# idra-lab/safe-mpc

Hardware: AMD Instinct MI355X
Metric: RTI-MPC instance-steps/s (batch=4096 per GPU, Z1 N=30) (higher is better)
Workload: dtype f64; 1 GPU; C1: Z1-class 6-DoF, N=30, 4096 instances/GPU, controller st (soft terminal NN row, MLP 12-256-256-256-1 fp32), EXT cost exact Hessian, 6 capsule pairs, Halton x0; batch_per_gpu=4096, batch_total=4096, horizon=30, controller=st, streams_per_gpu=3, qp_form=throughput, hip_graphs=False

## Files before the change

include/smpc.h:

```cpp
#ifndef SMPC_H_
#define SMPC_H_

#include <stddef.h>
#include <stdint.h>

#ifdef __cplusplus
extern "C" {
#endif

#define SMPC_ABI_VERSION 5

#define SMPC_MAX_NQ 7
#define SMPC_MAX_NX 14
#define SMPC_MAX_POINTS 12
#define SMPC_MAX_ROWS 12
#define SMPC_MAX_LAYERS 6
#define SMPC_MAX_N 63
#define SMPC_NP 5

#define SMPC_INF 1.0e5

#define SMPC_OK 0
#define SMPC_EINVAL (-1)
#define SMPC_ENOMEM (-2)
// ... 90 lines not shown
} smpc_problem_desc;

typedef struct {
    double tau[SMPC_MAX_NQ];
    double M[SMPC_MAX_NQ * SMPC_MAX_NQ];
    double dtau_dq[SMPC_MAX_NQ * SMPC_MAX_NQ];
    double dtau_dv[SMPC_MAX_NQ * SMPC_MAX_NQ];
    double ee[3];
    double cost_grad_q[SMPC_MAX_NQ];
    double cost_hess_qq[SMPC_MAX_NQ * SMPC_MAX_NQ];
    double row_val[SMPC_MAX_ROWS];
    double row_grad[SMPC_MAX_ROWS * SMPC_MAX_NQ];
    double nn_val;
    double nn_grad[SMPC_MAX_NX];
} smpc_node_eval;

typedef struct smpc_handle smpc_handle;

int smpc_create(const smpc_problem_desc* desc, int device, smpc_handle** out);
void smpc_destroy(smpc_handle* h);
int smpc_abi_version(void);
const char* smpc_last_error(const smpc_handle* h);

int smpc_set_mlp(smpc_handle* h, int nlayers, const int32_t* dims, const float* const* W, const float* const* b,
                 int on_device);
enum { SMPC_ACT_GELU_TANH = 0, SMPC_ACT_RELU = 1, SMPC_ACT_ELU = 2, SMPC_ACT_TANH = 3, SMPC_ACT_SILU = 4 };
int smpc_set_mlp_activation(smpc_handle* h, int act);

int smpc_set_horizon(smpc_handle* h, int N);

enum { SMPC_QP_AUTO = -1, SMPC_QP_THROUGHPUT = 0, SMPC_QP_LATENCY = 1 };
int smpc_set_qp_mode(smpc_handle* h, int mode);

int smpc_set_stage_bounds(smpc_handle* h, const double* lo, const double* hi);

int smpc_set_instance_bounds(smpc_handle* h, int B, const double* lo, const double* hi, int on_device);

#define SMPC_SCENE_ROW 8
int smpc_set_instance_scene(smpc_handle* h, int B, const double* geom, int on_device);

int smpc_set_instance_scene_track(smpc_handle* h, int B, int64_t T, const double* geom, int on_device);

int smpc_set_scene_clock(smpc_handle* h, const int64_t* d_clock);

int smpc_set_instance_world_track(smpc_handle* h, int B, int64_t T, const double* geom, int on_device);

enum { SMPC_FORECAST_HOLD = 0, SMPC_FORECAST_CV = 1, SMPC_FORECAST_TRUE = 2 };
int smpc_forecast_scene(smpc_handle* h, int B, int mode, int n_sel, const int32_t* select);

int smpc_set_instance_observed_track(smpc_handle* h, int B, int64_t T, const double* geom, int on_device);

#define SMPC_FIT_MAX 32
int smpc_forecast_scene_fit(smpc_handle* h, int B, int window, int n_sel, const int32_t* select);

int smpc_set_instance_curves(smpc_handle* h, int B, int64_t L, const double* curves, int on_device);

int smpc_set_instance_models(smpc_handle* h, int B, const smpc_joint* joints, int on_device);

int smpc_set_mlp_context(smpc_handle* h, int n_ctx, const float* Wc, const double* ctx_mean, const double* ctx_std,
                         const double* ctx_default, int on_device);

int smpc_set_instance_context(smpc_handle* h, int B, const double* ctx, int on_device);

int smpc_set_instance_context_track(smpc_handle* h, int B, int64_t T, const double* ctx, int on_device);

int smpc_set_slack_weights(smpc_handle* h, const double* zl);
// ... 194 lines not shown
```

safe_mpc_amd/_lib.py:

```python
from __future__ import annotations

import ctypes as C
import os
import subprocess

from .problem import Joint, NodeEval, ProblemDesc

_CSRC = os.path.join(os.path.dirname(os.path.abspath(__file__)), 'csrc')
LIB_PATH = os.environ.get('SMPC_HIP_LIB') or os.path.join(_CSRC, 'libsmpc_hip.so')

SYMBOLS = ['smpc_create', 'smpc_destroy', 'smpc_abi_version', 'smpc_last_error', 'smpc_set_mlp', 'smpc_set_horizon',
           'smpc_set_stage_bounds', 'smpc_set_slack_weights', 'smpc_set_instance_bounds', 'smpc_solve_batch', 'smpc_eval_nodes', 'smpc_guess_correction',
           'smpc_provide_control', 'smpc_check_trajectory', 'smpc_plant_step', 'smpc_rollout_batch', 'smpc_sync', 'smpc_stream',
           'smpc_enable_timing', 'smpc_get_timing', 'smpc_get_qp_timing', 'smpc_get_qp_wave_stats', 'smpc_policy_step', 'smpc_loop_pre',
           'smpc_loop_post', 'smpc_loop_apply_backup', 'smpc_loop_classify_aborts', 'smpc_get_timing_history',
           'smpc_accumulate_stats', 'smpc_set_mlp_activation', 'smpc_set_qp_mode', 'smpc_merit_terms', 'smpc_sqp_batch', 'smpc_check_guess',
           'smpc_score_rollout', 'smpc_set_instance_scene', 'smpc_ik_batch', 'smpc_ray_update', 'smpc_set_instance_curves',
           'smpc_set_instance_scene_track', 'smpc_set_scene_clock', 'smpc_set_mlp_context', 'smpc_set_instance_context',
           'smpc_set_instance_models', 'smpc_set_instance_context_track', 'smpc_set_instance_world_track', 'smpc_forecast_scene',
           'smpc_set_instance_observed_track', 'smpc_forecast_scene_fit']


class EngineError(RuntimeError):
    pass


_vp = C.c_void_p


class PolicyParams(C.Structure):
    _fields_ = [('kind', C.c_int32), ('abort_flag', C.c_int32), ('collision_first_node', C.c_int32), ('reserved0', C.c_int32),
                ('tol_x', C.c_double), ('alpha', C.c_double), ('tol_safe', C.c_double), ('tube', C.c_double),
                ('x_min', _vp), ('x_max', _vp), ('row_lb_chk', _vp), ('row_ub_chk', _vp), ('stage_lo', _vp), ('stage_hi', _vp)]


class PolicyState(C.Structure):
    _fields_ = [(k, _vp) for k in ('x_guess', 'u_guess', 'x_temp', 'u_temp', 'p', 'x_viable', 'fails', 'current_step', 'r',
                                   'status', 'qp_iter', 'traj')] + [('traj_len', C.c_int64)]


class LoopState(C.Structure):
    _fields_ = [(k, _vp) for k in ('x_cur', 'alive', 'sa', 'collided', 'ja', 'last_x', 'last_u', 'x_abort', 'u_abort', 'step',
                                   'x_log', 'u_log', 'r_log', 'resumed')]


class SqpOpts(C.Structure):
    _fields_ = [('max_iter', C.c_int32), ('reserved0', C.c_int32), ('tol', C.c_double), ('armijo', C.c_double),
                ('alpha_reduction', C.c_double), ('alpha_min', C.c_double), ('mu0', C.c_double), ('mu_max', C.c_double)]

# ... 75 lines not shown
    L.smpc_set_instance_world_track.argtypes = [vp, C.c_int, C.c_int64, dp, C.c_int]
    L.smpc_forecast_scene.argtypes = [vp, C.c_int, C.c_int, C.c_int, dp]
    L.smpc_set_instance_observed_track.argtypes = [vp, C.c_int, C.c_int64, dp, C.c_int]
    L.smpc_forecast_scene_fit.argtypes = [vp, C.c_int, C.c_int, C.c_int, dp]
    L.smpc_set_instance_curves.argtypes = [vp, C.c_int, C.c_int64, dp, C.c_int]
    L.smpc_solve_batch.argtypes = [vp, C.c_int, dp, dp, dp, dp, dp, dp, dp, dp, C.c_int]
    L.smpc_eval_nodes.argtypes = [vp, C.c_int, dp, dp, dp, dp, C.c_int]
    L.smpc_guess_correction.argtypes = [vp, C.c_int, dp, dp, C.c_int]
    L.smpc_provide_control.argtypes = [vp, C.c_int, dp, dp, dp, dp, dp, dp, C.c_int]
    L.smpc_check_trajectory.argtypes = [vp, C.c_int, C.c_int, dp, dp, dp, C.c_double, dp, dp, C.c_double, C.c_double,
                                        dp, dp, C.c_int]
    L.smpc_plant_step.argtypes = [vp, C.c_int, dp, dp, dp, dp, dp, dp, C.c_int]
    L.smpc_rollout_batch.argtypes = [vp, C.c_int, C.c_int, dp, dp, dp, dp, dp, dp, dp, dp, dp, dp, C.c_int]
    L.smpc_sync.argtypes = [vp]
    L.smpc_stream.argtypes = [vp]
    L.smpc_stream.restype = C.c_void_p
    L.smpc_enable_timing.argtypes = [vp, C.c_int]
    L.smpc_get_timing.argtypes = [vp, C.POINTER(C.c_float)]
    L.smpc_get_qp_timing.argtypes = [vp, C.POINTER(C.c_float)]
    L.smpc_get_qp_wave_stats.argtypes = [vp, C.POINTER(C.c_double)]
    L.smpc_policy_step.argtypes = [vp, C.c_int, C.POINTER(PolicyParams), C.POINTER(PolicyState), dp, dp, dp, dp, dp, dp]
    L.smpc_loop_pre.argtypes = [vp, C.c_int, C.c_int, C.POINTER(LoopState), dp, dp, dp, dp]
    L.smpc_loop_apply_backup.argtypes = [vp, C.c_int, C.c_int, C.POINTER(LoopState), C.c_int, dp, dp, dp, dp, dp, dp, dp]
    L.smpc_loop_post.argtypes = [vp, C.c_int, C.POINTER(PolicyParams), C.POINTER(LoopState), dp, dp, dp]
    L.smpc_loop_classify_aborts.argtypes = [vp, C.c_int, C.POINTER(LoopState), C.c_int, dp, dp]
    L.smpc_get_timing_history.argtypes = [vp, C.c_int, C.POINTER(C.c_float)]
    L.smpc_accumulate_stats.argtypes = [vp, C.c_int, dp, dp, dp]
    L.smpc_set_mlp_activation.argtypes = [vp, C.c_int]
    L.smpc_set_mlp_context.argtypes = [vp, C.c_int, dp, dp, dp, dp, C.c_int]
    L.smpc_set_instance_context.argtypes = [vp, C.c_int, dp, C.c_int]
    L.smpc_set_instance_context_track.argtypes = [vp, C.c_int, C.c_int64, dp, C.c_int]
    L.smpc_set_instance_models.argtypes = [vp, C.c_int, dp, C.c_int]
    L.smpc_set_qp_mode.argtypes = [vp, C.c_int]
    L.smpc_merit_terms.argtypes = [vp, C.c_int, dp, dp, dp, dp, dp, dp, dp, dp, dp, C.c_int]
    L.smpc_sqp_batch.argtypes = [vp, C.c_int, C.POINTER(SqpOpts), dp, dp, dp, dp, C.POINTER(SqpState), C.c_int]
    L.smpc_check_guess.argtypes = [vp, C.c_int, dp, dp, C.POINTER(GuessCheck), dp, dp, dp, C.c_int]
    L.smpc_score_rollout.argtypes = [vp, C.c_int, C.c_int, dp, dp, dp, dp, C.POINTER(ScoreParams), dp, dp, dp, C.c_int]
    L.smpc_ik_batch.argtypes = [vp, C.c_int, C.c_int, dp, dp, C.POINTER(IkParams), dp, dp, dp, dp, C.c_int]
    L.smpc_ray_update.argtypes = [vp, C.c_int, C.POINTER(RayOpts), C.POINTER(RayState), C.POINTER(SqpState), dp, dp, dp, dp, dp, C.c_int]
    _lib = L
    return L
```

safe_mpc_amd/csrc/engine.hip:

```cpp
#include <hip/hip_runtime.h>

#include <cstdarg>
#include <cstdio>
#include <cstring>
#include <new>
#include <type_traits>
#include <vector>

#include "../../include/smpc.h"
#include "kernel_qp.hpp"
#include "kernel_qp_wg.hpp"
#include "kernel_build.hpp"
#include "kernels_callers.hpp"
#include "kernels_policy.hpp"
#include "kernels_mlp.hpp"
#include "kernels_nodes.hpp"
#include "kernels_sqp.hpp"
#include "kernels_guess.hpp"
#include "kernels_score.hpp"
#include "kernels_ik.hpp"
#include "kernels_rays.hpp"
#include "kernels_forecast.hpp"

using namespace smpc;
// ... 58 lines not shown
    smpc_problem_desc desc;
    int device = 0;
    int N = 0;
    hipStream_t stream = nullptr;
    smpc_problem_desc* d_desc = nullptr;
    DevBuf<double> d_lo, d_hi;
    DevBuf<double> d_zl;
    InstSlot<double> bounds{"per-instance bounds", "smpc_set_instance_bounds"};
    InstSlot<double> scene{"instance scene", "smpc_set_instance_scene"};
    int64_t scene_T = 1;
    const int64_t* scene_clock = nullptr;
    bool scene_fc = false;
    InstSlot<double> world{"instance world track", "smpc_set_instance_world_track"};
    int64_t world_T = 1;
    InstSlot<double> seen{"instance observed track", "smpc_set_instance_observed_track"};
    int64_t seen_T = 1;
    InstSlot<double> curves{"instance curve table", "smpc_set_instance_curves"};
    int64_t curves_L = 0;
    InstSlot<float> ctx{"instance context", "smpc_set_instance_context"};
    int64_t ctx_T = 1;
    bool ctx_fc = false;
    InstSlot<smpc_joint> models{"instance model table", "smpc_set_instance_models"};
    Net own_net;
    const Net* net = &own_net;
    DevBuf<double> d_ev;
    DevBuf<double> d_nn;
    DevBuf<double> d_ws;
    int qp_mode = -2;
    DevBuf<double> d_hrec;
    bool wg_lds_raised[2] = {false, false};
    DevBuf<int32_t> d_order, d_last_it;
    int order_B = 0;
    DevBuf<int32_t> d_ord_hist;
    DevBuf<float> d_S, d_y, d_GS, d_dA, d_dB;
    DevBuf<int32_t> d_nn_idx;
    int32_t* d_nn_cnt = nullptr;
    DevBuf<float> d_act[SMPC_MAX_LAYERS];
    DevBuf<float> d_dg[SMPC_MAX_LAYERS];
    DevBuf<char> d_stage;
    ParamBlock chk{"check bounds"};
    ParamBlock gchk{"guess check bounds"};
    ParamBlock schk{"score bounds"};
    ParamBlock ikb{"inverse kinematics bounds"};
    DevBuf<char> d_roll;
    int timing = 0;
    int timed = 0;
    static constexpr int EV_RING = 64;
    hipEvent_t ev_sets[EV_RING][5] = {};
    bool ev_complete[EV_RING] = {};
    hipEvent_t* ev_t = ev_sets[0];
    int ev_cur = 0;
    bool timing_now = false;
    long timed_count = 0;
    std::vector<smpc_handle*> kids;
    hipEvent_t ev_fork = nullptr, ev_join = nullptr;
    DevBuf<unsigned long long> d_wstat;
    const uint8_t* d_active = nullptr;
    DevBuf<char> d_polw;
    float last_ms[4] = {0, 0, 0, 0};
    long mlp_rows_whole = 0;
    long mlp_rows_hint = 0;
    DevBuf<char> d_par;
    DevBuf<char> d_sqp;
    DevBuf<int32_t> d_guess;
    DevBuf<char> d_score;
    char err[256] = "";
// ... 345 lines not shown
    }
    if (st->traj) {
        if (st->traj_len < 1) return fail(h, SMPC_EINVAL, "traj_len must be >= 1");
        *out = TrajSrc{st->traj, (long)st->traj_len, 0};
    }
    return SMPC_OK;
}

template <int NQ>
int launch_eval(smpc_handle* h, int B, const double* d_xg, const double* d_ug, const double* d_p, double* d_ev) {
    const int N = h->N;
    hipStream_t s = h->stream;
    const long n1 = (long)B * (N + 1);
    with_scene(h, B, [&](auto SCENE, auto sc) {
        return with_model(h, B, [&](auto MODEL, auto... md) {
            hipLaunchKernelGGL((k_node_linearise<NQ, SCENE, MODEL>), dim3((unsigned)((n1 + 63) / 64)), dim3(64), 0, s, h->d_desc, B, N, d_xg,
                               d_ug, d_p, d_ev, sc, md...);
            return SMPC_OK;
        });
    });
    HIPCHK(h, hipGetLastError());
    int rc;
    if ((rc = launch_nn<NQ>(h, B, d_xg, d_p, d_ev, 0))) return rc;
    if (h->desc.nn_mode == SMPC_NN_ALL && h->d_nn_cnt) HIPCHK(h, hipMemsetAsync(h->d_nn_cnt, 0, sizeof(int32_t), s));
    return SMPC_OK;
}

constexpr size_t qp_nt_threshold = (size_t)384 << 20;
static int qp_nt_mode() {
    static const int v = [] { const char* e = getenv("SMPC_QP_NT"); return e ? atoi(e) : -1; }();
    return v;
}

template <class F> int with_rows(const smpc_handle* h, F&& f) {
    switch (h->desc.n_rows) {
    case 6: return f(std::integral_constant<int, 6>{});
    case 4: return f(std::integral_constant<int, 4>{});
    default: return f(std::integral_constant<int, -1>{});
    }
}

int ensure_instance_bounds(smpc_handle* h, int B, bool zero) { return h->bounds.room(h, (size_t)2 * B * (h->N + 1) * 2 * h->desc.nq, zero); }
double* instance_hi(const smpc_handle* h) { return h->bounds.d.p ? h->bounds.d.p + h->bounds.d.cap / (2 * sizeof(double)) : nullptr; }

struct StageBounds {
    const double *lo, *hi;
    long stride;
};
StageBounds stage_bounds(const smpc_handle* h, int B) {
    if (const double* lo = h->bounds.for_batch(B)) return {lo, instance_hi(h), (long)(h->N + 1) * 2 * h->desc.nq};
    return {h->d_lo.p, h->d_hi.p, 0L};
}

template <int NQ>
int launch_stage_records(smpc_handle* h, int B, const double* x0, const double* xg, const double* ug, const double* p, bool timed) {
    int rc;
    if ((rc = launch_nn<NQ>(h, B, xg, p, h->d_nn.p, h->desc.nn_mode == SMPC_NN_TERMINAL ? 2 : 1))) return rc;
    if (timed) HIPCHK(h, hipEventRecord(h->ev_t[1], h->stream));
    const StageBounds bd = stage_bounds(h, B);
    const long nodes = (long)B * (h->N + 1);
    const dim3 grd((unsigned)((nodes + 64 / SB_G - 1) / (64 / SB_G))), blk(64);
    const double* nn = h->desc.nn_mode != SMPC_NN_NONE ? h->d_nn.p : nullptr;
    int32_t* const zero_cnt = h->desc.nn_mode == SMPC_NN_ALL ? h->d_nn_cnt : nullptr;
    with_rows(h, [&](auto MR) {
        return with_scene(h, B, [&](auto SCENE, auto sc) {
            return with_model(h, B, [&](auto MODEL, auto... md) {
// ... 93 lines not shown
        h->timing_now = !capturing(h);
    }
    const bool timed = h->timing_now;
    if (timed) {
        h->ev_cur = (h->ev_cur + 1) % smpc_handle::EV_RING;
        h->ev_t = h->ev_sets[h->ev_cur];
        h->ev_complete[h->ev_cur] = false;
        h->timed_count++;
        HIPCHK(h, hipEventRecord(h->ev_t[0], h->stream));
    }
    if ((rc = launch_stage_records<NQ>(h, B, x0, xg, ug, p, timed))) return rc;
    const int wg_nhw = qp_wg_choice<NQ>(h, B);
    const bool wg = wg_nhw > 0;
    const int32_t* order = nullptr;
    if (h->order_B == B && B > 1 && !wg) {
        hipLaunchKernelGGL(k_order_by_iters, dim3((B + ORD_PER_BLOCK - 1) / ORD_PER_BLOCK), dim3(64), 0, h->stream, B, h->d_last_it.p,
                           h->d_order.p, h->d_ord_hist.p, h->d_ord_hist.p + 256, h->d_ord_hist.p + 512);
        order = h->d_order.p;
    } else {
        HIPCHK(h, hipMemsetAsync(h->d_ord_hist.p, 0, 520 * sizeof(int32_t), h->stream));
    }
    unsigned long long* wstat = nullptr;
    if (timed && h->timing == 1) {
        const unsigned long long init[4] = {0ull, ~0ull, 0ull, 0ull};
        HIPCHK(h, hipMemcpyAsync(h->d_wstat.p, init, sizeof(init), hipMemcpyHostToDevice, h->stream));
        wstat = h->d_wstat.p;
    }
    if (wg) {
        if ((rc = wg_nhw == 8 ? launch_qp_wg<NQ, 8>(h, B, x0, xg, ug, xo, uo, st, it) : launch_qp_wg<NQ, 4>(h, B, x0, xg, ug, xo, uo, st, it))) return rc;
    } else {
        const bool nt = qp_nt_mode() < 0 ? ws_doubles_per_instance(h, h->N) * sizeof(double) * (size_t)B >= qp_nt_threshold : qp_nt_mode() > 0;
        with_rows(h, [&](auto MR) {
            const auto launch = [&](auto NT) {
                hipLaunchKernelGGL((k_qp_ipm<NQ, MR, NT>), dim3((B + 1) / 2), dim3(64), 0, h->stream, h->d_desc, B, h->N, x0, xg, ug, h->d_ws.p,
                                   xo, uo, st, it, order, h->d_last_it.p, wstat, h->d_active, h->d_ord_hist.p);
                return SMPC_OK;
            };
            if constexpr (MR < 0) return launch(std::false_type{});
            else return nt ? launch(std::true_type{}) : launch(std::false_type{});
        });
    }
    h->order_B = B;
    HIPCHK(h, hipGetLastError());
    if (timed) {
        HIPCHK(h, hipEventRecord(h->ev_t[3], h->stream));
        h->ev_complete[h->ev_cur] = true;
        h->timed = 1;
    }
    return SMPC_OK;
}

struct ChkBlock { double *x_min, *x_max, *row_lb, *row_ub; size_t doubles; };
ChkBlock chk_block(double* base, int nq) {
    Carve m = dense(base);
    ChkBlock b{};
    b.x_min = m.take<double>(2 * nq);
    b.x_max = m.take<double>(2 * nq);
    b.row_lb = m.take<double>(SMPC_MAX_ROWS);
    b.row_ub = m.take<double>(SMPC_MAX_ROWS);
    b.doubles = m.off / sizeof(double);
    return b;
}
int upload_check_bounds(smpc_handle* h, const double* x_min, const double* x_max, const double* row_lb_chk,
                        const double* row_ub_chk) {
    const int nq = h->desc.nq, nr = h->desc.n_rows;
    std::vector<double> img(chk_block(nullptr, nq).doubles, 0.0);
    const ChkBlock b = chk_block(img.data(), nq);
    put(b.x_min, x_min, 2 * nq);
// ... 65 lines not shown
    return SMPC_OK;
}

struct RollScratch {
    int32_t *fails, *accept, *it;
    double *xo, *uo;
    size_t bytes;
};
RollScratch roll_layout(char* base, int n, int N, int nq) {
    Carve m{base};
    RollScratch r{};
    r.fails = m.take<int32_t>(n);
    r.accept = m.take<int32_t>(n);
    r.xo = m.take<double>((size_t)n * (N + 1) * 2 * nq);
    r.uo = m.take<double>((size_t)n * N * nq);
    r.it = m.take<int32_t>(n);
    r.bytes = m.off;
    return r;
}

int rollout_workers(smpc_handle* h, int n) {
    while ((int)h->kids.size() < n) {
        smpc_handle* k = nullptr;
        int rc = smpc_create(&h->desc, h->device, &k);
        if (rc) return fail(h, rc, "rollout worker: %s", smpc_last_error(nullptr));
        h->kids.push_back(k);
    }
    for (int i = 0; i < n; i++) {
        smpc_handle* k = h->kids[i];
        int rc;
        if (k->N != h->N && (rc = smpc_set_horizon(k, h->N))) return fail(h, rc, "rollout worker: %s", k->err);
        k->net = h->net;
        k->qp_mode = h->qp_mode;
        const size_t nb = (size_t)(h->N + 1) * 2 * h->desc.nq;
        HIPCHK(h, hipMemcpyAsync(k->d_lo.p, h->d_lo.p, nb * sizeof(double), hipMemcpyDeviceToDevice, k->stream));
        HIPCHK(h, hipMemcpyAsync(k->d_hi.p, h->d_hi.p, nb * sizeof(double), hipMemcpyDeviceToDevice, k->stream));
        if (h->d_zl.p) {
            if ((rc = k->d_zl.reserve(k, "slack weights", sizeof(double) * (h->N + 1)))) return fail(h, rc, "rollout worker: %s", k->err);
            HIPCHK(h, hipMemcpyAsync(k->d_zl.p, h->d_zl.p, sizeof(double) * (h->N + 1), hipMemcpyDeviceToDevice, k->stream));
        } else if (k->d_zl.p) {
            HIPCHK(h, hipStreamSynchronize(k->stream));
            k->d_zl.release();
        }
    }
    return SMPC_OK;
}

struct ParScratch {
    double *p1, *x0, *xg, *ug, *p, *xo, *uo;
    int32_t *st, *it, *ok, *safe, *list, *pos, *n_open;
    uint8_t* active;
    size_t bytes;
};
ParScratch par_layout(char* base, int B, int N, int nq) {
    const size_t S = (size_t)B * (N - 1), nx = 2 * (size_t)nq;
    Carve m{base};
    ParScratch c{};
    c.p1 = m.take<double>((size_t)B * (N + 1) * SMPC_NP);
    c.x0 = m.take<double>(S * nx);
    c.xg = m.take<double>(S * (N + 1) * nx);
    c.ug = m.take<double>(S * N * nq);
    c.p = m.take<double>(S * (N + 1) * SMPC_NP);
    c.xo = m.take<double>(S * (N + 1) * nx);
    c.uo = m.take<double>(S * N * nq);
    c.st = m.take<int32_t>(S);
    c.it = m.take<int32_t>(S);
// ... 585 lines not shown
        for (size_t i = 0; i < n; i++) {
            if (!(ctx[i] - ctx[i] == 0.0)) {
                const size_t bt = i / nc;
                if (T == 1) return fail(h, SMPC_EINVAL, "context of instance %zu (of B=%d), number %zu (of %d) is not finite", bt, B, i % nc, nc);
                return fail(h, SMPC_EINVAL, "context track of instance %zu (of B=%d), column %zu (of T=%lld), number %zu (of %d) is not finite",
                            bt / (size_t)T, B, bt % (size_t)T, (long long)T, i % nc, nc);
            }
            norm[i] = (float)((ctx[i] - net.ctx_mean[i % nc]) / net.ctx_std[i % nc]);
        }
    }
    int rc;
    if ((rc = h->ctx.room(h, n))) return rc;
    if (on_device) {
        CtxNorm nm;
        for (int c = 0; c < MLP_KPAD; c++) { nm.mean[c] = net.ctx_mean[c]; nm.std[c] = net.ctx_std[c]; }
        hipLaunchKernelGGL(k_ctx_normalise, dim3((unsigned)((n + 63) / 64)), dim3(64), 0, h->stream, (long)n, nc, ctx, nm, h->ctx.d.p);
        HIPCHK(h, hipGetLastError());
    } else if ((rc = h->ctx.upload(h, norm.data(), n, false)))
        return rc;
    h->ctx.commit(B);
    h->ctx_T = T;
    h->ctx_fc = false;
    return SMPC_OK;
}

int smpc_set_instance_context(smpc_handle* h, int B, const double* ctx, int on_device) {
    return smpc_set_instance_context_track(h, B, 1, ctx, on_device);
}

int smpc_set_qp_mode(smpc_handle* h, int mode) {
    if (!h) return SMPC_EINVAL;
    if (mode < SMPC_QP_AUTO || mode > SMPC_QP_LATENCY) return fail(h, SMPC_EINVAL, "qp mode %d (SMPC_QP_AUTO, _THROUGHPUT, _LATENCY)", mode);
    h->qp_mode = mode;
    return SMPC_OK;
}

int smpc_set_horizon(smpc_handle* h, int N) {
    if (!h) return SMPC_EINVAL;
    if (N < 1 || N > SMPC_MAX_N) return fail(h, SMPC_EINVAL, "N=%d outside 1..%d", N, SMPC_MAX_N);
    (void)hipSetDevice(h->device);
    HIPCHK(h, hipStreamSynchronize(h->stream));
    h->N = N;
    h->bounds.clear();
    drop_forecast(h);
    h->order_B = 0;
    for (DevBuf<double>* buf : {&h->d_zl, &h->bounds.d, &h->d_ev, &h->d_nn, &h->d_ws, &h->d_hrec}) buf->release();
    h->d_par.release();
    h->d_sqp.release();
    h->d_guess.release();
    return upload_bounds(h, nullptr, nullptr);
}

int smpc_set_stage_bounds(smpc_handle* h, const double* lo, const double* hi) {
    if (!h) return SMPC_EINVAL;
    if ((lo == nullptr) != (hi == nullptr)) return fail(h, SMPC_EINVAL, "lo and hi must both be given or both be NULL");
    (void)hipSetDevice(h->device);
    return upload_bounds(h, lo, hi);
}

int smpc_set_slack_weights(smpc_handle* h, const double* zl) {
    if (!h) return SMPC_EINVAL;
    (void)hipSetDevice(h->device);
    HIPCHK(h, hipStreamSynchronize(h->stream));
    if (!zl) {
        h->d_zl.release();
        return SMPC_OK;
// ... 997 lines not shown
    if (h->timing != 1 || !h->timed || !h->d_wstat.p) return fail(h, SMPC_ESTATE, "no solve has been timed since smpc_enable_timing(1)");
    (void)hipSetDevice(h->device);
    HIPCHK(h, hipStreamSynchronize(h->stream));
    unsigned long long w[4];
    HIPCHK(h, hipMemcpy(w, h->d_wstat.p, sizeof(w), hipMemcpyDeviceToHost));
    const double tick_us = 1e-2;
    out3[0] = w[3] ? (double)w[0] / (double)w[3] * tick_us : 0.0;
    out3[1] = w[3] ? (double)(w[2] - w[1]) * tick_us : 0.0;
    out3[2] = (double)w[3];
    return SMPC_OK;
}

}

extern "C" int smpc_debug_scene_slots(smpc_handle* h, double* scene_out, size_t scene_cap, float* ctx_out, size_t ctx_cap, int64_t* info) {
    if (!h || !info) return SMPC_EINVAL;
    (void)hipSetDevice(h->device);
    HIPCHK(h, hipStreamSynchronize(h->stream));
    const size_t ns = (size_t)h->scene.B * (size_t)h->scene_T * h->desc.n_rows * SMPC_SCENE_ROW;
    const size_t nc = (size_t)h->ctx.B * (size_t)h->ctx_T * h->net->n_ctx;
    const int64_t inf[6] = {h->scene.B, h->scene_T, h->scene.B && h->scene_fc, h->ctx.B, h->ctx_T, h->ctx.B && h->ctx_fc};
    memcpy(info, inf, sizeof(inf));
    if (scene_out && ns) {
        if (ns > scene_cap) return fail(h, SMPC_EINVAL, "smpc_debug_scene_slots: the scene holds %zu doubles, room for %zu", ns, scene_cap);
        HIPCHK(h, hipMemcpy(scene_out, h->scene.d.p, ns * sizeof(double), hipMemcpyDeviceToHost));
    }
    if (ctx_out && nc) {
        if (nc > ctx_cap) return fail(h, SMPC_EINVAL, "smpc_debug_scene_slots: the context holds %zu floats, room for %zu", nc, ctx_cap);
        HIPCHK(h, hipMemcpy(ctx_out, h->ctx.d.p, nc * sizeof(float), hipMemcpyDeviceToHost));
    }
    return SMPC_OK;
}

extern "C" int smpc_debug_stage_records(smpc_handle* h, int B, const double* x0, const double* xg, const double* ug, const double* p,
                                        int path, double* ws_out, int32_t* layout) {
    if (!h || B <= 0 || !x0 || !xg || !ug || !p || !ws_out || !layout) return SMPC_EINVAL;
    (void)hipSetDevice(h->device);
    int rc;
    if ((rc = guard_scene_context_and_models(h, B, "smpc_debug_stage_records"))) return rc;
    if ((rc = ensure_batch(h, B))) return rc;
    const int N = h->N, nx = 2 * h->desc.nq, nu = h->desc.nq;
    Stage io{h, false};
    const double *dx0, *dxg, *dug, *dp;
    if ((rc = io.place([&](Stage& v) {
             dx0 = v.in(x0, (size_t)B * nx);
             dxg = v.in(xg, (size_t)B * (N + 1) * nx);
             dug = v.in(ug, (size_t)B * N * nu);
             dp = v.in(p, (size_t)B * (N + 1) * SMPC_NP);
         })))
        return rc;
    const size_t per = ws_doubles_per_instance(h, N);
    HIPCHK(h, hipMemsetAsync(h->d_ws.p, 0, per * (size_t)B * sizeof(double), h->stream));
    (void)&launch_stage_records<5>, (void)&launch_stage_records_per_node<5>;
    (void)&launch_stage_records<6>, (void)&launch_stage_records_per_node<6>;
    (void)&launch_stage_records<7>, (void)&launch_stage_records_per_node<7>;
    if ((rc = with_nq(h, [&](auto NQ) {
             return path == 1 ? launch_stage_records<NQ>(h, B, dx0, dxg, dug, dp, false) : launch_stage_records_per_node<NQ>(h, B, dx0, dxg, dug, dp);
         })))
        return rc;
    HIPCHK(h, hipMemcpyAsync(ws_out, h->d_ws.p, per * (size_t)B * sizeof(double), hipMemcpyDeviceToHost, h->stream));
    if ((rc = io.finish())) return rc;
    return with_nq(h, [&](auto NQ) {
        const QpLayout<NQ> Ly(h->desc.n_rows);
        const int v[24] = {Ly.stride, Ly.nIMG, Ly.oIMG, Ly.oSL, Ly.nF, Ly.oR0, Ly.oR1, Ly.oR2, Ly.oCZA, Ly.oCZN, Ly.oZ, Ly.oZN, Ly.NRT, Ly.nJ,
                           (int)per, 12, Ly.iTT, Ly.iGT, Ly.iGN, Ly.iB, Ly.iSC, Ly.iHQQ, Ly.iGZ, 0};
        for (int i = 0; i < 24; i++) layout[i] = v[i];
// ... 19 lines not shown
```

safe_mpc_amd/csrc/kernel_qp.hpp:

```cpp
#pragma once
#include <type_traits>

#include "device_model.hpp"

namespace smpc {

constexpr double QP_THR = 1e-1;
constexpr double QP_THR_HARD = 3e-2;
constexpr double QP_FTB = 0.995;
constexpr double QP_ALPHA_MIN = 1e-12;
constexpr double QP_ABSENT = 1e300;

constexpr int qp_even_c(int n) { return (n + 1) & ~1; }
constexpr int qp_al8(int n) { return (n + 7) & ~7; }

template <int NQ> struct QpLayout {
    static constexpr int NX = 2 * NQ, NU = NQ, NZ = 3 * NQ;
    static constexpr int NZP = qp_even_c(NZ), NQP = qp_even_c(NQ), WS2 = qp_even_c(NX + 1);
    static constexpr int LC0 = WS2;
    static constexpr int KS = qp_even_c(LC0 + NQ);
    static constexpr int WR = NX + 1, LOFF = NQ * WR, NWP = qp_even_c(LOFF + NQ * (NQ + 1) / 2);
    __host__ __device__ static constexpr int w_coff(int j) { return LOFF + j * NQ - j * (j - 1) / 2; }
    int MR, MRP, NRC, NRT;
    int iTT, iGT, iGN, iHQQ, iGZ, iB, iSC, nIMG;
// ... 392 lines not shown
        *(w + Ly.oCZN + hl) = 0.0;
        sE[r] = -(ll - lu);
    }
    if (hl < 4) *(w + Ly.oSL + hl) = hl == 0 ? wsoft : (hl == 1 ? bflag : 0.0);
    if (hl < 8) *(w + Ly.oWC + hl) = 0.0;
    if (hl < NZ) { *(w + Ly.oZ + hl) = sZ0[hl]; *(w + Ly.oZN + hl) = sZ0[hl]; }
    lds_fence();
    if (hl < NZ && !(k == 0 && hl >= NU) && !(last && hl < NU)) {
        double a = sGZ[hl];
        for (int r = 0; r < NRC; r++) a = fma(sC[r * NZP + hl], sE[NX + r], a);
        if (hl >= NU) a += sE[hl - NU];
        r0_loc = fmax(r0_loc, fabs(a));
    }
    if (!last && hl < NX) {
        double ax = 0.0;
        if (k == 0) ax = hl < NQ ? sZ0[NU + hl] + dt * sZ0[NU + NQ + hl] : sZ0[NU + hl];
        r0_loc = fmax(r0_loc, fabs(ax + sB[hl]));
    }
    double inf0 = 0.0;
    if (k == 0 && D->rows_at_node0 && hl >= rC0 && hl < rNN) {
        const smpc_row& row = D->rows[hl - rC0];
        double v = e.row_val[hl - rC0];
        for (int c = 0; c < NZ; c++) v = fma(sC[(hl - NX) * NZP + c], sZ0[c], v);
        if ((fabs(row.lb) < SMPC_INF && v < row.lb - D->qp_tol) || (fabs(row.ub) < SMPC_INF && v > row.ub + D->qp_tol)) inf0 = 1.0;
    }
    const double R0 = half_max(r0_loc), musum = half_sum(mu_acc), cntsum = half_sum((double)cnt), infs = half_max(inf0);
    if (hl < 4) w[Ly.oPART + hl] = hl == 0 ? R0 : (hl == 1 ? musum : (hl == 2 ? cntsum : infs));
}

#ifndef QP_WAVES_PER_EU
#define QP_WAVES_PER_EU 2
#endif

template <int NQ, int MRT, bool NT>
__global__ __launch_bounds__(64) __attribute__((amdgpu_waves_per_eu(QP_WAVES_PER_EU, QP_WAVES_PER_EU))) void k_qp_ipm(
    const smpc_problem_desc* __restrict__ D, int B, int N, const double* __restrict__ x0, const double* __restrict__ xg,
    const double* __restrict__ ug, double* __restrict__ ws_all, double* __restrict__ x_out, double* __restrict__ u_out,
    int32_t* __restrict__ status, int32_t* __restrict__ qp_iter, const int32_t* __restrict__ order,
    int32_t* __restrict__ last_iter, unsigned long long* __restrict__ wstat, const uint8_t* __restrict__ active,
    int32_t* __restrict__ it_hist) {
    using LyT = QpLayout<NQ>;
    constexpr int NX = 2 * NQ, NU = NQ, NZ = 3 * NQ, NZP = LyT::NZP, NQP = LyT::NQP, WS2 = LyT::WS2, NL = 32,
                  LC0 = LyT::LC0, KS = LyT::KS, NWP = LyT::NWP;
    auto ldnt = [](auto* p) {
        if constexpr (NT) return __builtin_nontemporal_load(p);
        else return *p;
    };
    auto stnt_b1 = [](auto v, auto* p) {
        if constexpr (NT) __builtin_nontemporal_store(v, p);
        else *p = v;
    };
    __shared__ unsigned long long s_tbegin[2];
    if (wstat && (threadIdx.x & 31) == 0) s_tbegin[threadIdx.x >> 5] = __builtin_amdgcn_s_memrealtime();
    constexpr int MR_MAX = MRT >= 0 ? MRT : SMPC_MAX_ROWS, MRP_MAX = qp_even_c(MR_MAX);
    constexpr int NRC_MAX = NQ + MR_MAX + 1;
    static_assert(MRT < 0 || NX + NRC_MAX <= NL, "one lane per constraint row");
    static_assert(KS <= NL, "one lane per column of [G | rho | I]");
    constexpr int NTRI_U = NQ * (NQ + 1) / 2, NTRI_X = NX * (NX + 1) / 2;
    constexpr int IMG_MAX = NZ * NQP + NQ * MRP_MAX + NX + qp_even_c(NQ * NQ) + NZP + NX + 4;
    constexpr int IMG_PF = (IMG_MAX / 2 + 31) / 32;
    constexpr int CST_MAX = NRC_MAX * NZP;
    constexpr int NF_MAX = NZ * NQP + NQ * MRP_MAX + NX + NX + 4, CST_PF = (NF_MAX / 2 + 31) / 32;
    constexpr int W_N2 = NWP / 2, WST_PF = (W_N2 + 31) / 32;
#ifdef QP_PROFILE
    unsigned long long tacc[16] = {0, 0, 0, 0, 0, 0, 0, 0, 0, 0, 0, 0, 0, 0, 0, 0};
    unsigned long long tprev = __builtin_readcyclecounter();
#endif
    const int hl = threadIdx.x & 31, half = threadIdx.x >> 5;
    const int slot = 2 * (int)blockIdx.x + half;
    if (slot >= B) return;
    const int b = order ? order[slot] : slot;
    if (active && !active[b]) {
        if (hl == 0) {
            status[b] = SMPC_STATUS_SUCCESS;
            if (qp_iter) qp_iter[b] = 0;
            if (last_iter) last_iter[b] = 0;
            if (it_hist) atomicAdd(&it_hist[0], 1);
        }
        return;
    }
    const LyT Ly(MRT >= 0 ? MRT : D->n_rows);
    const int MR = Ly.MR, MRP = Ly.MRP, NRC = Ly.NRC, NRT = Ly.NRT;
    const int rT0 = NX, rC0 = NX + NQ, rNN = NX + NQ + MR;
    double* const ws = ws_all + (size_t)b * Ly.per_instance(N);
    const double dt = D->dt, cB = 0.5 * dt * dt;
    const int img_n2 = Ly.nIMG >> 1;
    const int c_n2 = Ly.nF >> 1;

    constexpr int O_D = IMG_MAX, O_E = O_D + NL, O_TD = O_E + NL, O_GD = O_TD + NZ * NQP, O_LAM = O_GD + NQ * MRP_MAX,
                  O_G = O_LAM + qp_even_c(NQ * NQ), O_WT = O_G + NQ * WS2, O_PA = O_WT + (NX + 1) * NQP,
                  O_PB2 = O_PA + NX * NX,
                  O_PEND = O_PB2 + NX * NX, O_STG = O_TD + CST_MAX + 2 * NWP,
                  O_PVA = O_PEND > O_STG ? O_PEND : O_STG, O_PVB = O_PVA + NX, O_PB = O_PVB + NX,
                  O_ZU = O_PB + NX, O_XB = O_ZU + NQP, O_RHO = O_XB + 2 * NX, O_WV = O_RHO + NQP, HALF_D = O_WV + NQP;
    __shared__ __attribute__((aligned(16))) double smem[2 * HALF_D];
    constexpr int XP = (NTRI_X + 31) / 32;
    constexpr int LDS_CAP = (160 * 1024) / 8;
    constexpr bool PASS_TAB = NQ == 6 && 2 * HALF_D * 8 + 16 + XP * 32 * 32 <= LDS_CAP;
    __shared__ uint4 desc[PASS_TAB ? 2 * XP * 32 : 1];
    __shared__ unsigned char triUi[PASS_TAB ? 1 : NTRI_U], triUj[PASS_TAB ? 1 : NTRI_U], triXi[PASS_TAB ? 1 : NTRI_X],
        triXj[PASS_TAB ? 1 : NTRI_X];
    double* const sIMG = smem + half * HALF_D;
    double* const sTT = sIMG + Ly.iTT;
    double* const sGT = sIMG + Ly.iGT;
    double* const sGN = sIMG + Ly.iGN;
    double* const sHQQ = sIMG + Ly.iHQQ;
    double* const sGZ = sIMG + Ly.iGZ;
    double* const sB = sIMG + Ly.iB;
    double* const sSC = sIMG + Ly.iSC;
    double* const sTD = sIMG + O_TD;
    double* const sGD = sIMG + O_GD;
    double* const sD = sIMG + O_D;
    double* const sE = sIMG + O_E;
    double* const sLam = sIMG + O_LAM;
    double* const sG = sIMG + O_G;
    double* const sWT = sIMG + O_WT;
    double* const sWI = sIMG + O_LAM;
// ... 28 lines not shown
            desc[2 * e] = uint4{pk(i * NQP, j * NQP), pk(i, j), pk(i * NX + j, i * NX + jj), pk(ii * NX + j, ii * NX + jj)};
            int iu, ju;
            tri_x(min(e, NTRI_U - 1), iu, ju);
            desc[2 * e + 1] = uint4{pk(j * NX + i, iq * NQ + jq), pk(iq * MRP, jq * MRP), pk(iu * NQP, ju * NQP), pk(iu, ju)};
        }
    } else {
        for (int e = hl; e < NTRI_U; e += 32) {
            int i = 0, rem = e;
            while (rem >= NQ - i) { rem -= NQ - i; i++; }
            triUi[e] = (unsigned char)i;
            triUj[e] = (unsigned char)(i + rem);
        }
        for (int e = hl; e < NTRI_X; e += 32) {
            int i = 0, j;
            if (e < NTRI_U) {
                int rem = e;
                while (rem >= NQ - i) { rem -= NQ - i; i++; }
                j = i + rem;
            } else {
                int rem = e - NTRI_U;
                while (rem >= (i < NQ ? NQ : NX - i)) { rem -= (i < NQ ? NQ : NX - i); i++; }
                j = (i < NQ ? NQ : i) + rem;
            }
            triXi[e] = (unsigned char)i;
            triXj[e] = (unsigned char)j;
        }
    }
    auto at = [](auto* base, unsigned off) {
        using T = std::remove_pointer_t<decltype(base)>;
        if constexpr (std::is_const_v<T>) return reinterpret_cast<const double*>(reinterpret_cast<const char*>(base) + off);
        else return reinterpret_cast<double*>(reinterpret_cast<char*>(base) + off);
    };

    const double* xb0 = xg + (size_t)b * (N + 1) * NX;
    const double* ub0 = ug + (size_t)b * N * NU;
    const double dx0_reg = hl < NX ? x0[(size_t)b * NX + hl] - xb0[hl] : 0.0;
    const int hl_u = hl < NQ ? hl : NQ - 1;
    const int hl_x = hl < NX ? hl : NX - 1;
    const int hr = hl < NRT ? hl : NRT - 1;
    const bool row_live = hl < NRT;
    const int hl_c = hr >= NX ? hr - NX : 0;
    const int hz = hl < NZ ? hl : NZ - 1;
    const int hl_px = hz >= NU ? hz - NU : 0;
    const int hc = hl < KS ? hl : KS - 1;
    const bool soft_lane = (hr == rNN);
    const int wbase = hc <= NX ? hc * NQ
                               : ((hc < LC0 || hc - LC0 >= NQ) ? NWP - (LyT::LOFF + NQ * (NQ + 1) / 2) % 2
                                                                : LyT::w_coff(hc - LC0) - (hc - LC0));
    const int lbase = LyT::w_coff(hl_u) - hl_u;

    auto stage_ptr = [&](int k) -> double* {
        asm volatile("" : "+v"(k));
        return ws + (size_t)k * Ly.stride;
    };

    double Lr[NQ][NQ], Linv[NQ];
    auto chol_from_lds = [&](const double* A) -> bool {
        bool ok = true;
#pragma unroll
        for (int j = 0; j < NQ; j++) {
            double dsum = A[j * NQ + j];
#pragma unroll
            for (int t = 0; t < j; t++) dsum = fma(-Lr[j][t], Lr[j][t], dsum);
            ok = ok && (dsum > 0.0);
            const double inv = fast_rsqrt(dsum);
            Linv[j] = inv;
// ... 774 lines not shown
                    if (k < N) { u_out[((size_t)b * N + k) * NU + hl] = v; bad |= !(v == v); }
                } else if (hl < NZ) {
                    x_out[((size_t)b * (N + 1) + k) * NX + hl - NU] = v;
                    bad |= !(v == v);
                }
            }
        }
    }
    const bool any_bad = half_max(bad ? 1.0 : 0.0) > 0.0;
#ifdef QP_PROFILE
    QPT(12);
    if (hl == 0) {
        for (int i = 0; i < 14; i++) atomicAdd(&g_qp_prof[i], tacc[i]);
        atomicAdd(&g_qp_prof[14], 1ull);
        atomicAdd(&g_qp_prof[15], (unsigned long long)it);
    }
#endif
    if (wstat && hl == 0) {
        const unsigned long long t_end = __builtin_amdgcn_s_memrealtime(), t_begin = s_tbegin[half];
        atomicAdd(&wstat[0], t_end - t_begin);
        atomicMin(&wstat[1], t_begin);
        atomicMax(&wstat[2], t_end);
        atomicAdd(&wstat[3], 1ull);
    }
    if (hl == 0) {
        int stc = (st_code == 0 || st_code == 2) ? SMPC_STATUS_SUCCESS : SMPC_STATUS_QP_FAILURE;
        if (ws[Ly.oPART + 3] != 0.0) stc = SMPC_STATUS_QP_FAILURE;
        if (any_bad && stc == SMPC_STATUS_SUCCESS) stc = SMPC_STATUS_NAN;
        status[b] = stc;
        if (qp_iter) qp_iter[b] = it;
        if (last_iter) last_iter[b] = it;
        if (it_hist) atomicAdd(&it_hist[min(it, 255)], 1);
    }
}


constexpr int ORD_PER_BLOCK = 256;
__global__ __launch_bounds__(64) void k_order_by_iters(int B, const int32_t* __restrict__ last_iter, int32_t* __restrict__ order,
                                                       int32_t* __restrict__ hist, int32_t* __restrict__ cur, int32_t* __restrict__ ticket) {
    __shared__ int offs[256];
    const int t = threadIdx.x;
    {
        int h4[4], run = 0;
#pragma unroll
        for (int j = 3; j >= 0; j--) { h4[j] = hist[4 * t + j]; }
        int mine = h4[0] + h4[1] + h4[2] + h4[3];
        int incl = mine;
#pragma unroll
        for (int o = 1; o < 64; o <<= 1) {
            const int v = __shfl_down(incl, o);
            if (t + o < 64) incl += v;
        }
        run = incl - mine;
#pragma unroll
        for (int j = 3; j >= 0; j--) { offs[4 * t + j] = run; run += h4[j]; }
    }
    __syncthreads();
    const int i0 = blockIdx.x * ORD_PER_BLOCK;
#pragma unroll
    for (int j = 0; j < ORD_PER_BLOCK / 64; j++) {
        const int i = i0 + 64 * j + t;
        if (i < B) {
            const int v = min(max(last_iter[i], 0), 255);
            const int pos = offs[v] + atomicAdd(&cur[v], 1);
            if (pos < B) order[pos] = i;
        }
    }
    __threadfence();
    __syncthreads();
    if (t == 0) offs[0] = atomicAdd(ticket, 1);
    __syncthreads();
    if (offs[0] == (int)gridDim.x - 1) {
#pragma unroll
        for (int j = 0; j < 4; j++) { hist[4 * t + j] = 0; cur[4 * t + j] = 0; }
        if (t == 0) *ticket = 0;
    }
}

}
```

safe_mpc_amd/solver.py:

```python
from __future__ import annotations

import contextlib
import ctypes as C
import sys

import numpy as np

from . import _lib
from .problem import FORECAST_MODES, JOINT_DTYPE, NODE_EVAL_DTYPE, SCENE_ROW, OcpProblem


SCORE_SLOTS = ('cost', 'ee_err2', 'u2', 'ee_dist', 'coll_margin', 'box_margin', 'safe_min')
SCORE_INDEX_SLOTS = ('coll_step', 'coll_row', 'box_step', 'safe_step')
SCORE_ND, SCORE_NI = len(SCORE_SLOTS), len(SCORE_INDEX_SLOTS)


def _is_torch(a):
    return type(a).__module__.startswith('torch')


def pad_hidden_units(Ws, bs, to=256):
    n, H = len(Ws), Ws[0].shape[0]
    if n < 2 or H % 64 == 0 or any(w.shape[0] != H for w in Ws[:-1]):
        return Ws, bs
# ... 79 lines not shown
            Wcp = np.zeros((Ws[0].shape[0], n_ctx), np.float32)
            Wcp[:Wc.shape[0]] = Wc
            if ctx_default is None:
                sel = getattr(net, 'ctx_select', None)
                ctx_default = self.problem.context_default(sel) if sel else net.ctx_mean
            cm, cs, cd = (np.ascontiguousarray(a, np.float64).reshape(-1) for a in (net.ctx_mean, net.ctx_std, ctx_default))
            if cm.shape != (n_ctx,) or cs.shape != (n_ctx,) or cd.shape != (n_ctx,):
                raise ValueError(f'set_mlp: ctx_mean, ctx_std and ctx_default must have {n_ctx} entries')
            self._chk(self.L.smpc_set_mlp_context(self.h, n_ctx, Wcp.ctypes.data, cm.ctypes.data, cs.ctypes.data, cd.ctypes.data, 0))
        self.net = net

    def set_instance_context(self, ctx=None):
        n_ctx = int(getattr(self.net, 'n_ctx', 0)) if self.net is not None else 0
        if ctx is not None and (ctx.ndim != 2 or (n_ctx and ctx.shape[1] != n_ctx)):
            raise ValueError(f'set_instance_context: expected [B, {n_ctx}], got {tuple(ctx.shape)}')
        self._set_instance(self.L.smpc_set_instance_context, 'set_instance_context', [ctx], None if ctx is None else ctx.shape[1:])

    def set_instance_context_track(self, ctx=None):
        n_ctx = int(getattr(self.net, 'n_ctx', 0)) if self.net is not None else 0
        T = 1
        if ctx is not None:
            if ctx.ndim != 3 or (n_ctx and ctx.shape[2] != n_ctx):
                raise ValueError(f'set_instance_context_track: expected [B, T, {n_ctx}], got {tuple(ctx.shape)}')
            T = int(ctx.shape[1])
            if T < 1:
                raise ValueError('set_instance_context_track: a track has at least one time column')
        self._set_instance(self.L.smpc_set_instance_context_track, 'set_instance_context_track', [ctx],
                           None if ctx is None else ctx.shape[1:], T)

    QP_MODES = {'auto': -1, 'throughput': 0, 'latency': 1}

    def set_qp_mode(self, mode):
        self._chk(self.L.smpc_set_qp_mode(self.h, self.QP_MODES[mode] if isinstance(mode, str) else int(mode)))

    def set_horizon(self, N):
        self._chk(self.L.smpc_set_horizon(self.h, int(N)))
        self.N = int(N)

    def set_stage_bounds(self, lo=None, hi=None):
        if lo is None:
            self._chk(self.L.smpc_set_stage_bounds(self.h, None, None))
            return
        lo = np.ascontiguousarray(lo, np.float64)
        hi = np.ascontiguousarray(hi, np.float64)
        assert lo.shape == (self.N + 1, self.nx) and hi.shape == lo.shape
        self._chk(self.L.smpc_set_stage_bounds(self.h, lo.ctypes.data, hi.ctypes.data))

    def set_slack_weights(self, zl=None):
        if zl is None:
            self._chk(self.L.smpc_set_slack_weights(self.h, None))
            return
        zl = np.ascontiguousarray(zl, np.float64)
        assert zl.shape == (self.N + 1,)
        self._chk(self.L.smpc_set_slack_weights(self.h, zl.ctypes.data))

    def set_instance_bounds(self, lo=None, hi=None):
        self._set_instance(self.L.smpc_set_instance_bounds, 'set_instance_bounds', [None, None] if lo is None else [lo, hi],
                           (self.N + 1, self.nx))

    def set_instance_scene(self, geom=None):
        self._set_instance(self.L.smpc_set_instance_scene, 'set_instance_scene', [geom], (len(self.problem.rows), SCENE_ROW))

    def set_instance_scene_track(self, geom=None):
        T = 1
        if geom is not None:
            if geom.ndim != 4:
# ... 634 lines not shown
```

Before: 1.146 million instance-steps/s.

## Add persistent-crew QP kernel with atomic ticket work stealing over instance pairs

Turns the QP IPM kernel into a loop in which each workgroup takes further instance pairs from an atomic ticket once its current pair finishes. This applies to every configuration except the NQ=6 dynamic-row form. The launch grid size comes from a crew fraction, set by environment variable or API, with a default of 1.0, which launches one workgroup per pair. At the default the loop exits right away, so behaviour stays close to before, apart from extra code, opaque-register asm tricks that may raise register pressure, and a second ticket slot reset in the order kernel.

Measured after the change: 1.162 million instance-steps/s (median of 6 runs). 1.01x the previous value.

```diff
diff --git a/include/smpc.h b/include/smpc.h
--- a/include/smpc.h
+++ b/include/smpc.h
@@ -146,6 +146,8 @@
 enum { SMPC_QP_AUTO = -1, SMPC_QP_THROUGHPUT = 0, SMPC_QP_LATENCY = 1 };
 int smpc_set_qp_mode(smpc_handle* h, int mode);
 
+int smpc_set_qp_crew(smpc_handle* h, double fraction, int waves);
+
 int smpc_set_stage_bounds(smpc_handle* h, const double* lo, const double* hi);
 
 int smpc_set_instance_bounds(smpc_handle* h, int B, const double* lo, const double* hi, int on_device);
diff --git a/safe_mpc_amd/_lib.py b/safe_mpc_amd/_lib.py
--- a/safe_mpc_amd/_lib.py
+++ b/safe_mpc_amd/_lib.py
@@ -14,7 +14,7 @@
            'smpc_provide_control', 'smpc_check_trajectory', 'smpc_plant_step', 'smpc_rollout_batch', 'smpc_sync', 'smpc_stream',
            'smpc_enable_timing', 'smpc_get_timing', 'smpc_get_qp_timing', 'smpc_get_qp_wave_stats', 'smpc_policy_step', 'smpc_loop_pre',
            'smpc_loop_post', 'smpc_loop_apply_backup', 'smpc_loop_classify_aborts', 'smpc_get_timing_history',
-           'smpc_accumulate_stats', 'smpc_set_mlp_activation', 'smpc_set_qp_mode', 'smpc_merit_terms', 'smpc_sqp_batch', 'smpc_check_guess',
+           'smpc_accumulate_stats', 'smpc_set_mlp_activation', 'smpc_set_qp_mode', 'smpc_set_qp_crew', 'smpc_merit_terms', 'smpc_sqp_batch', 'smpc_check_guess',
            'smpc_score_rollout', 'smpc_set_instance_scene', 'smpc_ik_batch', 'smpc_ray_update', 'smpc_set_instance_curves',
            'smpc_set_instance_scene_track', 'smpc_set_scene_clock', 'smpc_set_mlp_context', 'smpc_set_instance_context',
            'smpc_set_instance_models', 'smpc_set_instance_context_track', 'smpc_set_instance_world_track', 'smpc_forecast_scene',
@@ -156,6 +156,8 @@
     L.smpc_set_instance_context_track.argtypes = [vp, C.c_int, C.c_int64, dp, C.c_int]
     L.smpc_set_instance_models.argtypes = [vp, C.c_int, dp, C.c_int]
     L.smpc_set_qp_mode.argtypes = [vp, C.c_int]
+    if hasattr(L, 'smpc_set_qp_crew'):
+        L.smpc_set_qp_crew.argtypes = [vp, C.c_double, C.c_int]
     L.smpc_merit_terms.argtypes = [vp, C.c_int, dp, dp, dp, dp, dp, dp, dp, dp, dp, C.c_int]
     L.smpc_sqp_batch.argtypes = [vp, C.c_int, C.POINTER(SqpOpts), dp, dp, dp, dp, C.POINTER(SqpState), C.c_int]
     L.smpc_check_guess.argtypes = [vp, C.c_int, dp, dp, C.POINTER(GuessCheck), dp, dp, dp, C.c_int]
diff --git a/safe_mpc_amd/csrc/engine.hip b/safe_mpc_amd/csrc/engine.hip
--- a/safe_mpc_amd/csrc/engine.hip
+++ b/safe_mpc_amd/csrc/engine.hip
@@ -114,6 +114,8 @@
     DevBuf<int32_t> d_order, d_last_it;
     int order_B = 0;
     DevBuf<int32_t> d_ord_hist;
+    double qp_crew = -1.0;
+    int qp_crew_waves = 0;
     DevBuf<float> d_S, d_y, d_GS, d_dA, d_dB;
     DevBuf<int32_t> d_nn_idx;
     int32_t* d_nn_cnt = nullptr;
@@ -525,6 +527,23 @@
     return v;
 }
 
+constexpr double QP_CREW_DEFAULT = 1.0;
+static double qp_crew_default() {
+    static const double v = [] {
+        const char* e = getenv("SMPC_QP_CREW");
+        const double f = e ? atof(e) : QP_CREW_DEFAULT;
+        return f > 0.0 && f <= 1.0 ? f : QP_CREW_DEFAULT;
+    }();
+    return v;
+}
+static int qp_crew_waves(const smpc_handle* h, int B) {
+    const int pairs = (B + 1) / 2;
+    if (h->qp_crew_waves > 0) return h->qp_crew_waves < pairs ? h->qp_crew_waves : pairs;
+    const double f = h->qp_crew > 0.0 ? h->qp_crew : qp_crew_default();
+    const int g = (int)ceil(f * pairs);
+    return g < 1 ? 1 : (g > pairs ? pairs : g);
+}
+
 template <class F> int with_rows(const smpc_handle* h, F&& f) {
     switch (h->desc.n_rows) {
     case 6: return f(std::integral_constant<int, 6>{});
@@ -684,8 +703,8 @@
         const bool nt = qp_nt_mode() < 0 ? ws_doubles_per_instance(h, h->N) * sizeof(double) * (size_t)B >= qp_nt_threshold : qp_nt_mode() > 0;
         with_rows(h, [&](auto MR) {
             const auto launch = [&](auto NT) {
-                hipLaunchKernelGGL((k_qp_ipm<NQ, MR, NT>), dim3((B + 1) / 2), dim3(64), 0, h->stream, h->d_desc, B, h->N, x0, xg, ug, h->d_ws.p,
-                                   xo, uo, st, it, order, h->d_last_it.p, wstat, h->d_active, h->d_ord_hist.p);
+                hipLaunchKernelGGL((k_qp_ipm<NQ, MR, NT>), dim3(qp_crew_form<NQ, MR>() ? qp_crew_waves(h, B) : (B + 1) / 2), dim3(64), 0, h->stream, h->d_desc, B, h->N, x0, xg, ug,
+                                   h->d_ws.p, xo, uo, st, it, order, h->d_last_it.p, wstat, h->d_active, h->d_ord_hist.p, h->d_ord_hist.p + 513);
                 return SMPC_OK;
             };
             if constexpr (MR < 0) return launch(std::false_type{});
@@ -817,6 +836,8 @@
         if (k->N != h->N && (rc = smpc_set_horizon(k, h->N))) return fail(h, rc, "rollout worker: %s", k->err);
         k->net = h->net;
         k->qp_mode = h->qp_mode;
+        k->qp_crew = h->qp_crew;
+        k->qp_crew_waves = h->qp_crew_waves;
         const size_t nb = (size_t)(h->N + 1) * 2 * h->desc.nq;
         HIPCHK(h, hipMemcpyAsync(k->d_lo.p, h->d_lo.p, nb * sizeof(double), hipMemcpyDeviceToDevice, k->stream));
         HIPCHK(h, hipMemcpyAsync(k->d_hi.p, h->d_hi.p, nb * sizeof(double), hipMemcpyDeviceToDevice, k->stream));
@@ -1468,6 +1489,15 @@
     if (!h) return SMPC_EINVAL;
     if (mode < SMPC_QP_AUTO || mode > SMPC_QP_LATENCY) return fail(h, SMPC_EINVAL, "qp mode %d (SMPC_QP_AUTO, _THROUGHPUT, _LATENCY)", mode);
     h->qp_mode = mode;
+    return SMPC_OK;
+}
+
+int smpc_set_qp_crew(smpc_handle* h, double fraction, int waves) {
+    if (!h) return SMPC_EINVAL;
+    if (waves < 0 || (waves == 0 && !(fraction > 0.0 && fraction <= 1.0)))
+        return fail(h, SMPC_EINVAL, "qp crew: fraction %g outside (0, 1], or %d wavefronts", fraction, waves);
+    h->qp_crew = waves > 0 ? -1.0 : fraction;
+    h->qp_crew_waves = waves;
     return SMPC_OK;
 }
 
@@ -2531,6 +2561,15 @@
     return SMPC_OK;
 }
 
+extern "C" int smpc_debug_qp_dispatch(smpc_handle* h, int32_t* out) {
+    if (!h || !out) return SMPC_EINVAL;
+    (void)hipSetDevice(h->device);
+    if (!h->d_ord_hist.p) return fail(h, SMPC_ESTATE, "smpc_debug_qp_dispatch: no solve yet");
+    HIPCHK(h, hipStreamSynchronize(h->stream));
+    HIPCHK(h, hipMemcpy(out, h->d_ord_hist.p, 520 * sizeof(int32_t), hipMemcpyDeviceToHost));
+    return SMPC_OK;
+}
+
 extern "C" int smpc_debug_stage_records(smpc_handle* h, int B, const double* x0, const double* xg, const double* ug, const double* p,
                                         int path, double* ws_out, int32_t* layout) {
     if (!h || B <= 0 || !x0 || !xg || !ug || !p || !ws_out || !layout) return SMPC_EINVAL;
diff --git a/safe_mpc_amd/csrc/kernel_qp.hpp b/safe_mpc_amd/csrc/kernel_qp.hpp
--- a/safe_mpc_amd/csrc/kernel_qp.hpp
+++ b/safe_mpc_amd/csrc/kernel_qp.hpp
@@ -448,13 +448,15 @@
 #define QP_WAVES_PER_EU 2
 #endif
 
+template <int NQ, int MRT> constexpr bool qp_crew_form() { return !(NQ == 6 && MRT < 0); }
+
 template <int NQ, int MRT, bool NT>
 __global__ __launch_bounds__(64) __attribute__((amdgpu_waves_per_eu(QP_WAVES_PER_EU, QP_WAVES_PER_EU))) void k_qp_ipm(
     const smpc_problem_desc* __restrict__ D, int B, int N, const double* __restrict__ x0, const double* __restrict__ xg,
     const double* __restrict__ ug, double* __restrict__ ws_all, double* __restrict__ x_out, double* __restrict__ u_out,
     int32_t* __restrict__ status, int32_t* __restrict__ qp_iter, const int32_t* __restrict__ order,
     int32_t* __restrict__ last_iter, unsigned long long* __restrict__ wstat, const uint8_t* __restrict__ active,
-    int32_t* __restrict__ it_hist) {
+    int32_t* __restrict__ it_hist, int32_t* __restrict__ ticket) {
     using LyT = QpLayout<NQ>;
     constexpr int NX = 2 * NQ, NU = NQ, NZ = 3 * NQ, NZP = LyT::NZP, NQP = LyT::NQP, WS2 = LyT::WS2, NL = 32,
                   LC0 = LyT::LC0, KS = LyT::KS, NWP = LyT::NWP;
@@ -467,7 +469,6 @@
         else *p = v;
     };
     __shared__ unsigned long long s_tbegin[2];
-    if (wstat && (threadIdx.x & 31) == 0) s_tbegin[threadIdx.x >> 5] = __builtin_amdgcn_s_memrealtime();
     constexpr int MR_MAX = MRT >= 0 ? MRT : SMPC_MAX_ROWS, MRP_MAX = qp_even_c(MR_MAX);
     constexpr int NRC_MAX = NQ + MR_MAX + 1;
     static_assert(MRT < 0 || NX + NRC_MAX <= NL, "one lane per constraint row");
@@ -482,23 +483,23 @@
     unsigned long long tacc[16] = {0, 0, 0, 0, 0, 0, 0, 0, 0, 0, 0, 0, 0, 0, 0, 0};
     unsigned long long tprev = __builtin_readcyclecounter();
 #endif
-    const int hl = threadIdx.x & 31, half = threadIdx.x >> 5;
-    const int slot = 2 * (int)blockIdx.x + half;
-    if (slot >= B) return;
-    const int b = order ? order[slot] : slot;
-    if (active && !active[b]) {
-        if (hl == 0) {
-            status[b] = SMPC_STATUS_SUCCESS;
-            if (qp_iter) qp_iter[b] = 0;
-            if (last_iter) last_iter[b] = 0;
-            if (it_hist) atomicAdd(&it_hist[0], 1);
-        }
-        return;
-    }
+    constexpr bool CREW = qp_crew_form<NQ, MRT>();
+    const smpc_problem_desc* __restrict__ const D_arg = D;
+    const int N_arg = N, n_pairs = (B + 1) >> 1;
+    int pair = (int)blockIdx.x;
+#pragma unroll 1
+    for (;;) {
+    int tid = (int)threadIdx.x, zero = 0;
+    if constexpr (CREW) {
+        asm volatile("" : "+v"(tid));
+        asm volatile("" : "+s"(zero));
+    }
+    const smpc_problem_desc* const D = D_arg + zero;
+    const int N = N_arg + zero;
+    const int hl = tid & 31, half = tid >> 5;
     const LyT Ly(MRT >= 0 ? MRT : D->n_rows);
     const int MR = Ly.MR, MRP = Ly.MRP, NRC = Ly.NRC, NRT = Ly.NRT;
     const int rT0 = NX, rC0 = NX + NQ, rNN = NX + NQ + MR;
-    double* const ws = ws_all + (size_t)b * Ly.per_instance(N);
     const double dt = D->dt, cB = 0.5 * dt * dt;
     const int img_n2 = Ly.nIMG >> 1;
     const int c_n2 = Ly.nF >> 1;
@@ -593,6 +594,21 @@
         else return reinterpret_cast<double*>(reinterpret_cast<char*>(base) + off);
     };
 
+    const int slot = 2 * pair + half;
+    bool live = slot < B;
+    const int b = live ? (order ? order[slot] : slot) : 0;
+    if (live && active && !active[b]) {
+        if (hl == 0) {
+            status[b] = SMPC_STATUS_SUCCESS;
+            if (qp_iter) qp_iter[b] = 0;
+            if (last_iter) last_iter[b] = 0;
+            if (it_hist) atomicAdd(&it_hist[0], 1);
+        }
+        live = false;
+    }
+    if (live) {
+    if (wstat && hl == 0) s_tbegin[half] = __builtin_amdgcn_s_memrealtime();
+    double* const ws = ws_all + (size_t)b * Ly.per_instance(N);
     const double* xb0 = xg + (size_t)b * (N + 1) * NX;
     const double* ub0 = ug + (size_t)b * N * NU;
     const double dx0_reg = hl < NX ? x0[(size_t)b * NX + hl] - xb0[hl] : 0.0;
@@ -1433,6 +1449,15 @@
         if (last_iter) last_iter[b] = it;
         if (it_hist) atomicAdd(&it_hist[min(it, 255)], 1);
     }
+    }
+    if constexpr (!CREW) break;
+    if ((int)gridDim.x >= n_pairs) break;
+    int nxt = 0;
+    if (tid == 0) nxt = atomicAdd(ticket, 1);
+    pair = (int)gridDim.x + __builtin_amdgcn_readfirstlane(nxt);
+    if (pair >= n_pairs) break;
+    lds_fence();
+    }
 }
 
 
@@ -1474,7 +1499,7 @@
     if (offs[0] == (int)gridDim.x - 1) {
 #pragma unroll
         for (int j = 0; j < 4; j++) { hist[4 * t + j] = 0; cur[4 * t + j] = 0; }
-        if (t == 0) *ticket = 0;
+        if (t == 0) { ticket[0] = 0; ticket[1] = 0; }
     }
 }
 
diff --git a/safe_mpc_amd/solver.py b/safe_mpc_amd/solver.py
--- a/safe_mpc_amd/solver.py
+++ b/safe_mpc_amd/solver.py
@@ -135,6 +135,9 @@
 
     def set_qp_mode(self, mode):
         self._chk(self.L.smpc_set_qp_mode(self.h, self.QP_MODES[mode] if isinstance(mode, str) else int(mode)))
+
+    def set_qp_crew(self, fraction=1.0, waves=0):
+        self._chk(self.L.smpc_set_qp_crew(self.h, float(fraction), int(waves)))
 
     def set_horizon(self, N):
         self._chk(self.L.smpc_set_horizon(self.h, int(N)))
```
